# SewoongLab/PLeaS-Merging

Measured on AMD Instinct MI355X. Metric: wall-clock (s): ResNet-101 pair, 100-batch act-match + 400-step PLeaS, 1/8 GPU, lower is better.
Workload: dtype f32

## Files before the change

### include/pleas_hip.h

```cpp
#ifndef PLEAS_HIP_H
#define PLEAS_HIP_H

#include <stddef.h>
#include <stdint.h>

#ifdef __cplusplus
extern "C" {
#endif

#define PLEAS_OK 0
#define PLEAS_EINVAL (-22)
#define PLEAS_ENOMEM (-12)
#define PLEAS_EHIP (-5)

const char* pleas_version(void);
const char* pleas_last_error(void);

#define PLEAS_EPI_INNER 0
#define PLEAS_EPI_NEG_CDIST 1
size_t pleas_gram_ws_bytes(int B, int C, int64_t HW);
int pleas_gram_accum(const float* x, const float* y, int B, int C, int64_t HW, int epilogue, int accumulate,
                     float* acc, void* ws, size_t ws_bytes, void* stream);

typedef struct pleas_gram_node {
// ... 90 lines not shown
    const float* ip;
    const float* w;
    const float* bias;
    const float* o1;
    const float* o2;
    const int32_t* row1;
    const int32_t* row2;
    float* resid;
    int N, Cout, Cin, Hin, Win, KH, KW, stride, pad, Csrc, n_merged;
    float dscale, loss_scale;
    int flags;
} pleas_fwd_layer;
#define PLEAS_FWD_KPOS_MAJOR 1
size_t pleas_fwd_batch_ws_bytes(const pleas_fwd_layer* layers, int n_layers);
int pleas_fwd_plan_lanes(double* form_ms, int* form_lane, int* form_items);
int pleas_fwd_plan_units(const pleas_fwd_layer* layers, int n_layers, const double* form_ms, int* units, int max_units);
int pleas_fwd_batch(const pleas_fwd_layer* layers, int n_layers, float* loss, void* ws, size_t ws_bytes, int ws_fresh,
                    void* stream);
int pleas_conv2d_fwd(const float* x, const float* w, const float* bias, float* y, int N, int Cin, int Hin, int Win, int Cout,
                     int KH, int KW, int stride, int pad, int flags, void* stream);
int pleas_conv2d_bn_act_fwd(const float* x, const float* w, const float* bias, float* y, const float* scale,
                            const float* shift, const float* res, float* z, int relu, int N, int Cin, int Hin, int Win,
                            int Cout, int KH, int KW, int stride, int pad, int flags, void* stream);
int pleas_conv2d_act_fwd(const float* x, const float* w, const float* bias, const float* scale, const float* shift,
                         const float* res, float* z, int relu, int N, int Cin, int Hin, int Win, int Cout, int KH, int KW,
                         int stride, int pad, int flags, void* stream);
size_t pleas_conv2d_bn_stats_ws_bytes(int N, int Cout, int Hout, int Wout, int batches);
int pleas_conv2d_bn_stats_fwd(const float* x, const float* w, const float* bias, float* y, int N, int Cin, int Hin, int Win,
                              int Cout, int KH, int KW, int stride, int pad, int flags, int batches, const float* gamma,
                              const float* beta, double eps, double momentum, float* running_mean, float* running_var,
                              int64_t* num_batches_tracked, float* scale, float* shift, void* ws, size_t ws_bytes, void* stream);
typedef struct pleas_wgrad_layer {
    const float* resid;
    const float* ip;
    float* grad;
    int N, Cout, Cin, Hin, Win, KH, KW, stride, pad;
    int flags;
} pleas_wgrad_layer;
#define PLEAS_WGRAD_ACCUMULATE 1
#define PLEAS_WGRAD_KPOS_MAJOR 2
int pleas_target_residual(const float* out, const float* o1, const float* o2, const int32_t* row1, const int32_t* row2,
                          int n_merged, int N, int C, int Csrc, int64_t HW, float dscale, float* resid, float* partials,
                          int* n_partials, void* stream);
int pleas_target_residual_max_partials(void);
int pleas_loss_final(const float* partials, const int* n_partials, const float* scale, int stride, int n_layers,
                     float* loss, void* stream);
// ... 38 lines not shown
```

### pleas_merging_amd/_lib.py

```python
from __future__ import annotations

import ctypes
import os
from ctypes import POINTER, c_char_p, c_float, c_int, c_int64, c_size_t, c_void_p
from typing import Optional

_LIB: Optional[ctypes.CDLL] = None
LIB_PATH = os.path.join(os.path.dirname(os.path.abspath(__file__)), "csrc", "libpleas_hip.so")

EPI_INNER, EPI_NEG_CDIST = 0, 1
ARITH_FP32, ARITH_SPLIT_BF16, ARITH_SPLIT_BF16_EXACT = 0, 1, 2
LSAP_MAX_N = 4096

SIGNATURES = {
    "pleas_version": (c_char_p, []),
    "pleas_last_error": (c_char_p, []),
    "pleas_gram_ws_bytes": (c_size_t, [c_int, c_int, c_int64]),
    "pleas_gram_accum": (c_int, [c_void_p, c_void_p, c_int, c_int, c_int64, c_int, c_int, c_void_p, c_void_p, c_size_t,
                                 c_void_p]),
    "pleas_lsap_batched": (c_int, [POINTER(c_void_p), POINTER(c_int), c_int, c_int, POINTER(c_void_p), c_void_p]),
    "pleas_lsap_host": (c_int, [c_void_p, c_int, c_int, c_int, c_void_p]),
    "pleas_bottleneck_ws_bytes": (c_size_t, [POINTER(c_int), c_int]),
    "pleas_bottleneck_batched": (c_int, [POINTER(c_void_p), POINTER(c_int), c_int, c_int, POINTER(c_void_p), c_void_p, c_void_p,
                                         c_size_t, c_void_p]),
# ... 30 lines not shown
    "pleas_prof_reset": (None, []),
    "pleas_prof_collect": (c_int, [c_int, POINTER(c_int64), POINTER(ctypes.c_double), POINTER(ctypes.c_double),
                                   POINTER(ctypes.c_double)]),
    "pleas_arith": (None, [c_int]),
    "pleas_arith_get": (c_int, []),
    "pleas_gram_batch_tune": (None, [c_int, c_int]),
    "pleas_target_residual": (c_int, [c_void_p, c_void_p, c_void_p, c_void_p, c_void_p, c_int, c_int, c_int, c_int,
                                      c_int64, c_float, c_void_p, c_void_p, POINTER(c_int), c_void_p]),
    "pleas_target_residual_max_partials": (c_int, []),
    "pleas_loss_final": (c_int, [c_void_p, c_void_p, c_void_p, c_int, c_int, c_void_p, c_void_p]),
    "pleas_cholesky_solve_batched": (c_int, [POINTER(c_void_p), POINTER(c_void_p), POINTER(c_int), POINTER(c_int), c_int,
                                             c_float, c_void_p, c_void_p]),
    "pleas_normal_eq_ws_bytes": (c_size_t, [c_void_p, c_int]),
    "pleas_normal_eq_accum": (c_int, [c_void_p, c_int, c_void_p, c_size_t, c_int, c_void_p]),
    "pleas_normal_eq_finalize": (c_int, [c_void_p, c_int, c_void_p]),
    "pleas_normal_eq_plan_info": (c_int, [c_void_p, c_int, c_void_p]),
    "pleas_fwd_batch_ws_bytes": (c_size_t, [c_void_p, c_int]),
    "pleas_fwd_plan_lanes": (c_int, [c_void_p, c_void_p, c_void_p]),
    "pleas_fwd_plan_units": (c_int, [c_void_p, c_int, c_void_p, c_void_p, c_int]),
    "pleas_allreduce_sum": (c_int, [c_void_p, c_int64, c_void_p, c_void_p]),
    "pleas_fwd_batch": (c_int, [c_void_p, c_int, c_void_p, c_void_p, c_size_t, c_int, c_void_p]),
    "pleas_conv2d_fwd": (c_int, [c_void_p, c_void_p, c_void_p, c_void_p] + [c_int] * 10 + [c_void_p]),
    "pleas_conv2d_bn_act_fwd": (c_int, [c_void_p] * 8 + [c_int] * 11 + [c_void_p]),
    "pleas_conv2d_act_fwd": (c_int, [c_void_p] * 7 + [c_int] * 11 + [c_void_p]),
    "pleas_conv2d_bn_stats_ws_bytes": (c_size_t, [c_int] * 5),
    "pleas_conv2d_bn_stats_fwd": (c_int, [c_void_p] * 4 + [c_int] * 11 + [c_void_p, c_void_p, ctypes.c_double, ctypes.c_double]
                                  + [c_void_p] * 6 + [c_size_t, c_void_p]),
    "pleas_pool_gather": (c_int, [c_void_p, c_void_p, c_void_p, c_int64, c_int, c_int64, c_int, c_void_p]),
    "pleas_top1_count": (c_int, [c_void_p, c_void_p, c_int64, c_int, c_void_p, c_void_p, c_void_p]),
    "pleas_softmax_xent": (c_int, [c_void_p, c_void_p, c_int64, c_int, c_float, c_void_p, c_void_p, c_void_p, c_void_p, c_void_p]),
    "pleas_wgrad_batch_ws_bytes": (c_size_t, [c_void_p, c_int]),
    "pleas_wgrad_batch": (c_int, [c_void_p, c_int, c_void_p, c_size_t, c_int, c_void_p]),
    "pleas_wgrad_plan_info": (c_int, [c_void_p, c_int, POINTER(c_int)]),
    "pleas_gram_batch_ws_bytes": (c_size_t, [c_void_p, c_int, POINTER(c_int), c_int]),
    "pleas_gram_batch": (c_int, [c_void_p, c_int, POINTER(c_void_p), POINTER(c_int), c_int, c_int, c_int, c_void_p,
                                 c_size_t, c_int, c_void_p]),
}


class MergeItem(ctypes.Structure):
    _fields_ = [("w1", c_void_p), ("w2", c_void_p), ("out", c_void_p), ("row1", c_void_p), ("row2", c_void_p),
                ("outer", c_int64), ("inner", c_int64), ("rows_out", c_int), ("rows_src", c_int), ("n_merged", c_int),
                ("sub_stride", c_int), ("sub_h", c_int), ("sub_w", c_int)]


class FwdLayer(ctypes.Structure):
# ... 50 lines not shown
```

### pleas_merging_amd/csrc/conv_fwd.hip

```cpp
#include <algorithm>
#include <mutex>
#include <vector>

#include "fwd_schedule.hpp"
#include "nt_tile.hpp"

namespace pleas {

typedef short s16x4_t __attribute__((ext_vector_type(4)));
typedef short s16x8_t __attribute__((ext_vector_type(8)));

constexpr int fTN = 128;

enum class FwdMode : int { Fit = 0, Conv = 1, ConvImage = 2, Image = 3, ConvStats = 4 };
constexpr int fModes = 5;
constexpr bool fwd_has_target(FwdMode m) { return m == FwdMode::Fit; }
constexpr bool fwd_has_image(FwdMode m) { return m == FwdMode::ConvImage || m == FwdMode::Image; }
constexpr bool fwd_stores_y(FwdMode m) { return m != FwdMode::Image; }
constexpr bool fwd_has_stats(FwdMode m) { return m == FwdMode::ConvStats; }

struct FwdLayerDev {
    const float* ip;
    const float* w;
    const float* bias;
    const float* o1;
    const float* o2;
    const int32_t* row1;
    const int32_t* row2;
    float* resid;
    int Cout, Cin, Hin, Win, Hout, Wout, KH, KW, stride, pad, Csrc, n_merged;
    uint32_t HWo, Ptot, Kd;
    float dscale;
    int variant;
    int part_base;
    int bn_relu;
    const float* bn_scale;
    const float* bn_shift;
    const float* bn_res;
    float* bn_z;
    double* st_part;
    uint32_t st_pb;
};
struct FwdItemDev {
    int layer, tm, tp, slot;
};

template <int TM, bool IMAGE>
struct FwdRowOps {
    int row1[TM / 8], row2[TM / 8];
    float bias[TM / 8];
};
template <int TM>
struct FwdRowOps<TM, true> {
    float scale[TM / 8], shift[TM / 8];
    float bias[TM / 8];
};
template <int TM, FwdMode MODE = FwdMode::Fit>
__device__ __forceinline__ void fwd_load_maps(const FwdLayerDev& L, const int i0, FwdRowOps<TM, fwd_has_image(MODE)>& ops) {
    const int tid = threadIdx.x;
#pragma unroll
    for (int j = 0; j < TM / 8; ++j) {
        const int co = min(i0 + (tid >> 5) + 8 * j, L.Cout - 1);
        if constexpr (fwd_has_image(MODE)) {
            ops.scale[j] = PLEAS_GLOBAL(L.bn_scale)[co];
            ops.shift[j] = PLEAS_GLOBAL(L.bn_shift)[co];
        } else {
            ops.row1[j] = L.row1 ? PLEAS_GLOBAL_I(L.row1)[co] : -1;
            ops.row2[j] = L.row2 ? PLEAS_GLOBAL_I(L.row2)[co] : -1;
        }
        ops.bias[j] = L.bias ? PLEAS_GLOBAL(L.bias)[co] : 0.f;
    }
}

template <int TM, FwdMode MODE = FwdMode::Fit>
__device__ __forceinline__ void fwd_epilogue(const FwdLayerDev& L, const FwdItemDev& it, f32x16 (&acc)[TM / 64][2],
                                             const FwdRowOps<TM, fwd_has_image(MODE)>& ops, float* smem, float* __restrict__ partials) {
    constexpr int MTM = TM / 64;
    constexpr int ROWS = TM / 8, GB = 8, NB = ROWS / GB;
    const int tid = threadIdx.x, lane = tid & 63, wave = tid >> 6;
    const int wm = wave >> 1, wn = wave & 1;
    const int i0 = it.tm * TM;
    const uint32_t p0 = (uint32_t)it.tp * fTN;
    constexpr int EL = 132;
    float* Ct = smem;
    auto spill_acc = [&]() {
#pragma unroll
        for (int sm = 0; sm < MTM; ++sm)
#pragma unroll
            for (int sn = 0; sn < 2; ++sn)
#pragma unroll
                for (int r = 0; r < 16; ++r) {
                    const int lco = wm * (TM / 2) + sm * 32 + (r & 3) + 8 * (r >> 2) + 4 * (lane >> 5);
                    Ct[lco * EL + wn * 64 + sn * 32 + (lane & 31)] = acc[sm][sn][r];
                }
        __syncthreads();
    };
    float sq = 0.f;
    constexpr int SPR = kThreads / TM;
    float st_bias = 0.f;
    if constexpr (fwd_has_stats(MODE)) st_bias = L.bias ? PLEAS_GLOBAL(L.bias)[min(i0 + tid / SPR, L.Cout - 1)] : 0.f;
    const bool vec_ok = (L.HWo % 4 == 0);
    const int pg = (tid & 31) * 4;
    const uint32_t Pg = p0 + pg;
    const bool gin = Pg < L.Ptot;
    const uint32_t gn = gin ? Pg / L.HWo : 0u, gp = gin ? Pg - gn * L.HWo : 0u;
    if (vec_ok) {
        f32x4 ta[NB][GB], tb[NB][GB];
        const uint32_t hw4 = 4u * L.HWo;
        const uint32_t gbase = 4u * (gn * (uint32_t)L.Csrc * L.HWo + gp);
        const uint32_t rbase = 4u * ((gn * (uint32_t)L.Cout + (uint32_t)i0 + (uint32_t)(tid >> 5)) * L.HWo + gp);
        const bool has_res = fwd_has_image(MODE) && L.bn_res != nullptr;
        const char* o1b = reinterpret_cast<const char*>(fwd_has_image(MODE) ? (has_res ? L.bn_res : L.ip) : L.o1);
        const char* o2b = reinterpret_cast<const char*>(L.o2);
        char* rb_ = reinterpret_cast<char*>(L.resid);
        char* zb_ = reinterpret_cast<char*>(L.bn_z);
        auto gather = [&](const int bt) {
#pragma unroll
            for (int u = 0; u < GB; ++u) {
                const int j = bt * GB + u;
                if constexpr (fwd_has_image(MODE)) {
                    const bool live = has_res && gin && i0 + (tid >> 5) + 8 * j < L.Cout;
                    const uint32_t oz = live ? rbase + (uint32_t)(8 * j) * hw4 : 0u;
                    const f32x4 idn = *(const __attribute__((address_space(1))) f32x4*)(o1b + oz);
                    ta[bt][u] = has_res ? idn : f32x4{0.f, 0.f, 0.f, 0.f};
                } else if constexpr (!fwd_has_target(MODE)) {
                    ta[bt][u] = tb[bt][u] = f32x4{0.f, 0.f, 0.f, 0.f};
                } else {
                    const uint32_t oa = (gin && ops.row1[j] >= 0) ? gbase + (uint32_t)ops.row1[j] * hw4 : 0u;
                    const uint32_t ob = (gin && ops.row2[j] >= 0) ? gbase + (uint32_t)ops.row2[j] * hw4 : 0u;
                    ta[bt][u] = *(const __attribute__((address_space(1))) f32x4*)(o1b + oa);
                    tb[bt][u] = *(const __attribute__((address_space(1))) f32x4*)(o2b + ob);
                }
            }
        };
        auto consume = [&](const int bt) {
#pragma unroll
            for (int u = 0; u < GB; ++u) {
                const int j = bt * GB + u;
                const int lco = (tid >> 5) + 8 * j, co = i0 + lco;
                const bool live = gin && co < L.Cout;
                if constexpr (fwd_has_image(MODE)) {
                    const f32x4 o = *reinterpret_cast<const f32x4*>(Ct + lco * EL + pg);
                    f32x4 y, z;
#pragma unroll
                    for (int e = 0; e < 4; ++e) {
                        y[e] = o[e] + ops.bias[j];
                        const float sm = fmaf(y[e], ops.scale[j], ops.shift[j]) + ta[bt][u][e];
                        z[e] = L.bn_relu ? fmaxf(sm, 0.f) : sm;
                    }
                    if (live) {
                        if constexpr (fwd_stores_y(MODE)) *(__attribute__((address_space(1))) f32x4*)(rb_ + (rbase + (uint32_t)(8 * j) * hw4)) = y;
                        *(__attribute__((address_space(1))) f32x4*)(zb_ + (rbase + (uint32_t)(8 * j) * hw4)) = z;
                    }
                } else {
                    const float coef = co < L.n_merged ? 0.5f : 1.0f;
                    const float ca = ops.row1[j] >= 0 ? coef : 0.f, cb = ops.row2[j] >= 0 ? coef : 0.f;
                    const f32x4 o = *reinterpret_cast<const f32x4*>(Ct + lco * EL + pg);
                    f32x4 d;
                    float s4 = 0.f;
#pragma unroll
                    for (int e = 0; e < 4; ++e) {
                        const float dd = (o[e] + ops.bias[j]) - fmaf(tb[bt][u][e], cb, ta[bt][u][e] * ca);
                        s4 = fmaf(dd, dd, s4);
                        d[e] = L.dscale * dd;
                    }
                    sq += live ? s4 : 0.f;
                    if (live) *(__attribute__((address_space(1))) f32x4*)(rb_ + (rbase + (uint32_t)(8 * j) * hw4)) = d;
                }
            }
        };
        gather(0);
        spill_acc();
        if constexpr (NB > 1) gather(1);
        consume(0);
        if constexpr (NB > 1) consume(1);
    } else {
        spill_acc();
#pragma unroll
        for (int j = 0; j < ROWS; ++j) {
            const int lco = (tid >> 5) + 8 * j, co = i0 + lco;
            if (co >= L.Cout || !gin) continue;
            const float coef = co < L.n_merged ? 0.5f : 1.0f;
            const f32x4 o = *reinterpret_cast<const f32x4*>(Ct + lco * EL + pg);
#pragma unroll
            for (int e = 0; e < 4; ++e) {
                const uint32_t Pe = Pg + e;
                if (Pe >= L.Ptot) break;
                const uint32_t n = Pe / L.HWo, p = Pe - n * L.HWo;
                if constexpr (fwd_has_image(MODE)) {
                    const size_t at = ((size_t)n * L.Cout + co) * L.HWo + p;
                    const float y = o[e] + ops.bias[j];
                    const float sm = fmaf(y, ops.scale[j], ops.shift[j]) + (L.bn_res ? PLEAS_GLOBAL(L.bn_res)[at] : 0.f);
                    if constexpr (fwd_stores_y(MODE)) PLEAS_GLOBAL_W(L.resid)[at] = y;
                    PLEAS_GLOBAL_W(L.bn_z)[at] = L.bn_relu ? fmaxf(sm, 0.f) : sm;
                } else {
                    float a = 0.f, b = 0.f;
                    if (ops.row1[j] >= 0) a = PLEAS_GLOBAL(L.o1)[((size_t)n * L.Csrc + ops.row1[j]) * L.HWo + p];
                    if (ops.row2[j] >= 0) b = PLEAS_GLOBAL(L.o2)[((size_t)n * L.Csrc + ops.row2[j]) * L.HWo + p];
                    const float dd = (o[e] + ops.bias[j]) - (a + b) * coef;
                    sq = fmaf(dd, dd, sq);
                    PLEAS_GLOBAL_W(L.resid)[((size_t)n * L.Cout + co) * L.HWo + p] = L.dscale * dd;
                }
            }
        }
    }
    if constexpr (fwd_has_stats(MODE)) {
        constexpr int NCH = 32 / SPR;
        const int r = tid / SPR, q = tid % SPR;
        const int skew = (NCH / 2) * (SPR == 2 ? q : q >> 1);
        const uint32_t bnext = (p0 / L.st_pb + 1u) * L.st_pb;
        const uint32_t n1 = min(L.Ptot - p0, (uint32_t)fTN), n0 = min(bnext - p0, n1);
        double a0 = 0.0, b0 = 0.0, a1 = 0.0, b1 = 0.0;
        const float* row = Ct + r * EL + q * NCH * 4;
        if (n0 == (uint32_t)fTN) {
#pragma unroll
            for (int i = 0; i < NCH; ++i) {
                const f32x4 o = *reinterpret_cast<const f32x4*>(row + 4 * ((i + skew) % NCH));
// ... 518 lines not shown
            } else {
                __syncthreads();
                store_b(0, rb0);
            }
        }
        __syncthreads();
        r1 = r2;
        cb1 = cb2;
    };
    int r = 0;
    int c = 0;
    for (; c + 2 < nchunks; c += 2) {
        const int ra_ = r1;
        step(c, r, ra1, ra0, rb1, rb0);
        const int rb_ = r1;
        step(c + 1, ra_, ra0, ra1, rb0, rb1);
        r = rb_;
    }
    if (c + 1 < nchunks) {
        const int ra_ = r1;
        step(c, r, ra1, ra0, rb1, rb0);
        r = ra_;
    }
    fwd_load_maps<TM, MODE>(L, i0, ops);
    compute((nchunks - 1) & 1, bsel, r);
    __syncthreads();
    fwd_epilogue<TM, MODE>(L, it, acc, ops, smem, partials);
}

struct FwdForm {
    bool flat;
    int tm;
    int sub;
    bool split;
    int occupancy[3];
    double weight;
};
constexpr int fForms = 10;
constexpr FwdForm kFwdForms[fForms] = {
    {false, 128, 4, false, {2, 2, 2}, 2.5}, {false, 64, 4, false, {2, 2, 2}, 2.5},
    {false, 128, 1, false, {2, 2, 2}, 2.5}, {false, 64, 1, false, {2, 2, 2}, 2.5},
    {true, 128, 0, true, {2, 2, 2}, 1.0},   {true, 128, 1, false, {2, 2, 2}, 2.0}, {true, 128, 2, true, {2, 2, 2}, 1.0},
    {true, 64, 0, true, {2, 3, 3}, 1.0},    {true, 64, 1, false, {2, 2, 2}, 2.0},  {true, 64, 2, true, {2, 3, 3}, 1.0},
};
constexpr int fwd_form_of(int variant) {
    if (variant & 8) return ((variant & 1) ? 7 : 4) + ((variant >> 4) & 3);
    return variant & 3;
}
constexpr bool fwd_forms_match_variants() {
    for (int f = 0; f < fForms; ++f) {
// ... 18 lines not shown
}
template <int FORM, int SPLIT, FwdMode MODE>
__global__ __launch_bounds__(kThreads, kFwdForms[FORM].occupancy[SPLIT]) void conv2d_fwd_kernel(const FwdLayerDev L, const int tms) {
    extern __shared__ __attribute__((aligned(16))) float smem[];
    const FwdItemDev it{0, (int)(blockIdx.x % (unsigned)tms), (int)(blockIdx.x / (unsigned)tms), 0};
    constexpr FwdForm F = kFwdForms[FORM];
    static_assert(!fwd_has_target(MODE), "the fit has its own kernel: tables of layers and items, loss partials");
    if constexpr (F.flat) fwd_flat_tile<F.tm, F.sub, SPLIT, MODE>(L, it, smem, nullptr);
    else fwd_tile<F.tm, F.sub, MODE>(L, it, smem, nullptr);
}
struct FwdFormKernels {
    void (*batch[3])(const FwdLayerDev*, const FwdItemDev*, float*);
    void (*conv2d[fModes][3])(const FwdLayerDev, const int);
};
template <int FORM>
static constexpr FwdFormKernels fwd_form_kernels() {
    constexpr int S = kFwdForms[FORM].split ? 1 : 0, S9 = kFwdForms[FORM].split ? 2 : 0;
    using M = FwdMode;
    return {{fwd_batch_kernel<FORM, 0>, fwd_batch_kernel<FORM, S>, fwd_batch_kernel<FORM, S9>},
            {{nullptr, nullptr, nullptr},
             {conv2d_fwd_kernel<FORM, 0, M::Conv>, conv2d_fwd_kernel<FORM, S, M::Conv>, conv2d_fwd_kernel<FORM, S9, M::Conv>},
             {conv2d_fwd_kernel<FORM, 0, M::ConvImage>, conv2d_fwd_kernel<FORM, S, M::ConvImage>, conv2d_fwd_kernel<FORM, S9, M::ConvImage>},
             {conv2d_fwd_kernel<FORM, 0, M::Image>, conv2d_fwd_kernel<FORM, S, M::Image>, conv2d_fwd_kernel<FORM, S9, M::Image>},
             {conv2d_fwd_kernel<FORM, 0, M::ConvStats>, conv2d_fwd_kernel<FORM, S, M::ConvStats>, conv2d_fwd_kernel<FORM, S9, M::ConvStats>}}};
}
static const FwdFormKernels kFwdKernels[fForms] = {fwd_form_kernels<0>(), fwd_form_kernels<1>(), fwd_form_kernels<2>(), fwd_form_kernels<3>(),
                                                   fwd_form_kernels<4>(), fwd_form_kernels<5>(), fwd_form_kernels<6>(), fwd_form_kernels<7>(),
                                                   fwd_form_kernels<8>(), fwd_form_kernels<9>()};
constexpr int fLanes = 3;
static SideStreams<fLanes> g_fwd_side;

struct FwdLossDev {
    int begin, count;
    float scale;
    int pad;
};
__global__ __launch_bounds__(64) void fwd_loss_kernel(const float* __restrict__ partials, const FwdLossDev* __restrict__ ld,
                                                      float* __restrict__ loss) {
    const FwdLossDev d = ld[blockIdx.x];
    double s = 0.0;
    for (int i = threadIdx.x; i < d.count; i += 64) s += (double)partials[d.begin + i];
#pragma unroll
    for (int off = 32; off >= 1; off >>= 1) s += __shfl_xor(s, off);
    if (threadIdx.x == 0) loss[blockIdx.x] = (float)(s * (double)d.scale);
}

constexpr int fPtrBatch = 56;
// ... 203 lines not shown
        units[4 * i + 1] = tmp.units[i].begin;
        units[4 * i + 2] = tmp.units[i].count;
        units[4 * i + 3] = tmp.units[i].lane;
    }
    return (int)tmp.units.size();
}

extern "C" size_t pleas_fwd_batch_ws_bytes(const pleas_fwd_layer* layers, int n_layers) {
    if (!layers || n_layers <= 0) return 0;
    FwdPlan tmp;
    if (build_fwd_plan(tmp, layers, n_layers) != PLEAS_OK) return 0;
    return tmp.total;
}

struct Conv2dCall {
    FwdMode mode;
    const float *x, *w, *bias;
    float* y;
    int N, Cin, Hin, Win, Cout, KH, KW, stride, pad, flags;
    void* stream;
    const float *scale = nullptr, *shift = nullptr, *res = nullptr;
    float* z = nullptr;
    int relu = 0;
};
struct Conv2dPlan { FwdLayerDev d; size_t lds = 0; int TM = 128; };

static int conv2d_describe(const Conv2dCall& c, Conv2dPlan& p) {
    FwdLayerDev& d = p.d;
    if (!c.x || !c.w || (!c.y && fwd_stores_y(c.mode))) return bad_arg("conv2d_fwd: null pointer");
    if (((uintptr_t)c.w & 15) != 0 || ((uintptr_t)c.x & 15) != 0)
        return bad_arg(fwd_has_stats(c.mode) ? "conv2d_bn_stats_fwd: x and w must be 16-byte aligned" : "conv2d_fwd: x and w must be 16-byte aligned");
    if (fwd_has_image(c.mode) && ((((uintptr_t)c.y | (uintptr_t)c.z | (uintptr_t)c.res) & 15) != 0))
        return bad_arg("conv2d_bn_act_fwd: y, z and res must be 16-byte aligned");
    pleas_fwd_layer l{};
    l.N = c.N; l.Cout = c.Cout; l.Cin = c.Cin; l.Hin = c.Hin; l.Win = c.Win; l.KH = c.KH; l.KW = c.KW; l.stride = c.stride; l.pad = c.pad;
    l.Csrc = 1; l.dscale = 1.f; l.flags = c.flags;
    d = FwdLayerDev{};
    if (const int rc = fwd_describe(l, d, p.lds, p.TM); rc != PLEAS_OK) return rc;
    d.ip = c.x; d.w = c.w; d.bias = c.bias; d.o1 = c.x; d.o2 = c.x; d.resid = c.y;
    d.bn_scale = c.scale; d.bn_shift = c.shift; d.bn_res = c.res; d.bn_z = c.z; d.bn_relu = c.relu ? 1 : 0;
    return PLEAS_OK;
}

static int conv2d_enqueue(const Conv2dCall& c, const Conv2dPlan& p) {
    const FwdLayerDev& d = p.d;
    const int tms = (int)ceil_div(c.Cout, p.TM), tps = (int)ceil_div((int64_t)d.Ptot, fTN);
    const dim3 grid((unsigned)((int64_t)tms * tps));
    hipStream_t st = (hipStream_t)c.stream;
    const double out_floats = (double)c.Cout * d.Ptot;
    ProfScope prof(kProfConv2d, 2.0 * c.Cout * (double)d.Kd * (double)d.Ptot,
                   ((double)c.Cin * c.N * c.Hin * c.Win + out_floats * ((c.mode == FwdMode::ConvImage ? 2.0 : 1.0) + (c.res ? 1.0 : 0.0))) * sizeof(float), st);
    hipLaunchKernelGGL(kFwdKernels[fwd_form_of(d.variant)].conv2d[(int)c.mode][arith_mode()], grid, dim3(kThreads), p.lds, st, d, tms);
    PLEAS_LAUNCH_CHECK("conv2d_fwd_kernel");
    return PLEAS_OK;
}

static int conv2d_launch(const Conv2dCall& c) {
    Conv2dPlan p;
    if (const int rc = conv2d_describe(c, p); rc != PLEAS_OK) return rc;
    return conv2d_enqueue(c, p);
}

extern "C" int pleas_conv2d_fwd(const float* x, const float* w, const float* bias, float* y, int N, int Cin, int Hin, int Win,
                                int Cout, int KH, int KW, int stride, int pad, int flags, void* stream_) {
    return conv2d_launch(Conv2dCall{FwdMode::Conv, x, w, bias, y, N, Cin, Hin, Win, Cout, KH, KW, stride, pad, flags, stream_});
}

extern "C" int pleas_conv2d_bn_act_fwd(const float* x, const float* w, const float* bias, float* y, const float* scale,
                                       const float* shift, const float* res, float* z, int relu, int N, int Cin, int Hin,
                                       int Win, int Cout, int KH, int KW, int stride, int pad, int flags, void* stream_) {
    if (!scale || !shift || !z) return bad_arg("conv2d_bn_act_fwd: null pointer");
    return conv2d_launch(Conv2dCall{FwdMode::ConvImage, x, w, bias, y, N, Cin, Hin, Win, Cout, KH, KW, stride, pad, flags, stream_,
                                    scale, shift, res, z, relu});
}

extern "C" int pleas_conv2d_act_fwd(const float* x, const float* w, const float* bias, const float* scale, const float* shift,
                                    const float* res, float* z, int relu, int N, int Cin, int Hin, int Win, int Cout, int KH,
                                    int KW, int stride, int pad, int flags, void* stream_) {
    if (!scale || !shift || !z) return bad_arg("conv2d_act_fwd: null pointer");
    return conv2d_launch(Conv2dCall{FwdMode::Image, x, w, bias, nullptr, N, Cin, Hin, Win, Cout, KH, KW, stride, pad, flags, stream_,
                                    scale, shift, res, z, relu});
}

static size_t conv_bn_stats_head(int Cout, int batches) { return (size_t)batches * Cout * 4; }

extern "C" size_t pleas_conv2d_bn_stats_ws_bytes(int N, int Cout, int Hout, int Wout, int batches) {
    if (N <= 0 || Cout <= 0 || Hout <= 0 || Wout <= 0 || batches <= 0) return 0;
    const int64_t tiles = ceil_div((int64_t)N * Hout * Wout, fTN);
    return (conv_bn_stats_head(Cout, batches) + (size_t)tiles * 2 * Cout * 2) * sizeof(double);
}

extern "C" int pleas_conv2d_bn_stats_fwd(const float* x, const float* w, const float* bias, float* y, int N, int Cin, int Hin, int Win,
                                         int Cout, int KH, int KW, int stride, int pad, int flags, int batches, const float* gamma,
                                         const float* beta, double eps, double momentum, float* running_mean, float* running_var,
                                         int64_t* num_batches_tracked, float* scale, float* shift, void* ws, size_t ws_bytes,
                                         void* stream_) {
// ... 135 lines not shown
```

### pleas_merging_amd/hip_ops.py

```python
from __future__ import annotations

import contextlib
import ctypes
import math
import os
import threading
from typing import List, Optional, Sequence, Tuple

import numpy as np
import torch

from . import _lib
from ._lib import ARITH_FP32, ARITH_SPLIT_BF16, ARITH_SPLIT_BF16_EXACT, EPI_INNER, EPI_NEG_CDIST, PleasHipError, check


class _Pinned(threading.local):

    depth = 0
    handle = 0


_PINNED = _Pinned()


# ... 745 lines not shown


def column_sum(x: torch.Tensor, out: torch.Tensor) -> torch.Tensor:
    _need_gpu(x, out)
    if x.dim() != 2 or not x.is_contiguous() or x.shape[0] < 1 or x.shape[1] < 1:
        raise PleasHipError("column_sum: x must be a contiguous, non-empty [N, C] tensor, got %s" % (tuple(x.shape),))
    if out.device != x.device or out.numel() != x.shape[1] or not out.is_contiguous():
        raise PleasHipError("column_sum: out must hold %d contiguous floats on x's device" % x.shape[1])
    check(_lib.lib().pleas_column_sum(x.data_ptr(), x.shape[0], x.shape[1], out.data_ptr(), _stream()), "pleas_column_sum")
    return out


def conv2d_bn_act(x: torch.Tensor, w: torch.Tensor, bias: Optional[torch.Tensor], stride: int, pad: int, kpos_major: bool,
                  scale: torch.Tensor, shift: torch.Tensor, res: Optional[torch.Tensor], relu: bool):
    operands, geometry, out_shape = _conv_call("conv2d_bn_act", x, w, bias, stride, pad, kpos_major, scale, shift)
    image = _image_operands("conv2d_bn_act", x, scale, shift, res, out_shape)
    y = torch.empty(out_shape, dtype=torch.float32, device=x.device)
    z = torch.empty_like(y)
    check(_lib.lib().pleas_conv2d_bn_act_fwd(*operands, y.data_ptr(), *image, z.data_ptr(), 1 if relu else 0, *geometry, _stream()),
          "pleas_conv2d_bn_act_fwd")
    return y, z


CONV_MAX_OUTPUT, CONV_MAX_PIXELS = 1 << 30, 1 << 31


def conv2d_sample_split(N: int, per_sample_out: int, pixels: int, limit: int = CONV_MAX_OUTPUT, align: int = 1) -> List[Tuple[int, int]]:
    if N <= 0:
        return []
    most = min((limit - 1) // per_sample_out, (CONV_MAX_PIXELS - 1) // pixels) // align * align
    if most <= 0:
        raise PleasHipError("conv2d_act: one sample (%d output elements, %d pixels) exceeds the per-call limit" % (per_sample_out, pixels))
    groups = -(-N // align)
    calls = -(-groups // (most // align))
    base, extra = divmod(groups, calls)
    parts, at = [], 0
    for i in range(calls):
        n = min((base + (1 if i < extra else 0)) * align, N - at)
        parts.append((at, n))
        at += n
    return parts


def conv2d_act(x: torch.Tensor, w: torch.Tensor, bias: Optional[torch.Tensor], stride: int, pad: int, kpos_major: bool,
               scale: torch.Tensor, shift: torch.Tensor, res: Optional[torch.Tensor], relu: bool,
               _limit: int = CONV_MAX_OUTPUT) -> torch.Tensor:
# ... 278 lines not shown
```

### pleas_merging_amd/methods/activation_matching.py

```python
from __future__ import annotations

import os

from typing import Callable, Dict, Iterable, List, Optional, Tuple

import torch
import torch.fx
from torch import nn

from ..core.solvers import hip_solve_lsa, hip_solve_minimax_assignment
from ..core.utils import Axis, Permutation, PermutationSpec
from .. import hip_ops
from ..hip_ops import cross_features_cdist, cross_features_inner_product

_FUSED_EPILOGUE = {}


def _register_fused():
    from .. import hip_ops

    _FUSED_EPILOGUE[hip_ops.cross_features_cdist] = hip_ops.EPI_NEG_CDIST
    _FUSED_EPILOGUE[hip_ops.cross_features_inner_product] = hip_ops.EPI_INNER


# ... 125 lines not shown
    return gm


def _bn_chains(traced: _Trace, model1: nn.Module, model2: nn.Module):
    from .source_forward import _foldable, _foldable_train, bn_chain

    mods1, mods2 = dict(model1.named_modules()), dict(model2.named_modules())
    at, absorbed, claimed = {}, set(), set()
    for node in traced.graph.nodes:
        if (node.op != "call_module" or len(node.args) != 1 or node.kwargs
                or not all(_foldable(m) or _foldable_train(m) for m in (mods1.get(node.target), mods2.get(node.target)))):
            continue
        add, relu, res = bn_chain(node, mods1, bare_add=True, claimed=claimed)
        last = relu or add or node
        at[last] = (node, add, relu, res)
        absorbed |= {n for n in (node, add, relu) if n is not None and n is not last}
    return at, absorbed


def _build_split_twin(model1: nn.Module, model2: nn.Module, axes: Iterable[Axis], emit: Callable, streams: _SideStream,
                      fuse_bn: bool = False, emit_derived: Optional[Callable] = None):
    import operator

    from .source_forward import _foldable, _train_fold, fold_bn

    traced = _Trace(model1)
    submods = dict(traced.named_modules())
    root = nn.ModuleList([model1, model2])
    chains, absorbed = _bn_chains(traced, model1, model2) if fuse_bn else ({}, set())
    want_early: Dict[str, List[int]] = {}
    for ax in axes:
        want_early.setdefault(ax.key, []).append(ax.axis)
    derivable = set()
    if emit_derived is not None:
        for bn, _add, _relu, _res in chains.values():
            src = bn.args[0]
            if isinstance(src, torch.fx.Node) and src.op not in ("placeholder", "output") and src not in absorbed \
                    and want_early.get(bn.name) == [1] and 1 in want_early.get(src.name, ()):
                derivable.add(bn)
    fold_attrs: Tuple[dict, dict] = ({}, {})
    want: Dict[str, List[int]] = {}
    for ax in axes:
        if ax.axis not in want.setdefault(ax.key, []):
            want[ax.key].append(ax.axis)
    twin = torch.fx.Graph()
    env = ({}, {})
    shared = {}
    for node in traced.graph.nodes:
        if node.op == "placeholder":
            shared[node] = twin.placeholder(node.target)
    ret = None
    for side in (1, 0):
        first = True
        for node in traced.graph.nodes:
            if node.op == "placeholder":
                env[side][node] = shared[node]
                if side == 1 and first:
                    env[side][node] = _node(twin, "call_function", streams.fork, (shared[node],), "fork")
                    first = False
                continue
            if node.op == "output":
                (ret,) = node.args
                continue
            if node in chains:
                bn, add, relu, res = chains[node]
                mod = (model1, model2)[side].get_submodule(bn.target)
                if _foldable(mod):
                    names = ["_pleas_%s_%d_%s" % (kind, side, bn.name) for kind in ("scale", "shift")]
                    for nm_, buf in zip(names, fold_bn(mod)):
                        root.register_buffer(nm_, buf, persistent=False)
                    attrs = (_node(twin, "get_attr", names[0], (), "bn_scale"), _node(twin, "get_attr", names[1], (), "bn_shift"))
                else:
                    fold = _node(twin, "call_function", _train_fold(mod, "%d_%s" % (side, bn.name), streams), (env[side][bn.args[0]],), "bn_stats")
                    attrs = (_node(twin, "call_function", operator.getitem, (fold, 0), "bn_scale"),
                             _node(twin, "call_function", operator.getitem, (fold, 1), "bn_shift"))
                fold_attrs[side][bn] = attrs
                fused = _node(twin, "call_function", hip_ops.bn_act_tracked,
                              (env[side][bn.args[0]], attrs[0], attrs[1], env[side][res] if res is not None else None,
                               relu is not None, bn not in derivable), "bn_chain")
                for slot, member in enumerate((bn, add, relu)):
                    if member is not None:
                        env[side][member] = _node(twin, "call_function", operator.getitem, (fused, slot), "chain_out")
                continue
            if node in absorbed:
                continue
            new = _out_of_place(twin, node, lambda n, side=side: env[side][n], submods)
            if new is not None:
                env[side][node] = new
                continue
            own = _own_conv(twin, node, side, (model1, model2)[side], env[side])
            if own is not None:
                env[side][node] = own
                continue
            new = twin.node_copy(node, lambda n, side=side: env[side][n])
            if node.op in ("call_module", "get_attr"):
                new.target = "%d.%s" % (side, node.target)
            env[side][node] = new
        if side == 1:
            _node(twin, "call_function", streams.back, (), "back")
    _node(twin, "call_function", streams.join, (), "join")
    cross: Dict[Tuple[str, int], torch.fx.Node] = {}
    for node in traced.graph.nodes:
        for a in want.get(node.name, ()) if node.op not in ("placeholder", "output") else ():
            if node in derivable:
                cross[node.name, a] = emit_derived(twin, node.name, node.args[0].name, a, fold_attrs[0][node], fold_attrs[1][node])
            else:
                cross[node.name, a] = emit(twin, node.name, a, env[0][node], env[1][node])
# ... 262 lines not shown
```

### pleas_merging_amd/methods/source_forward.py

```python
from __future__ import annotations

import operator
import os
from typing import Callable, Optional

import torch
import torch.fx
import torch.nn.functional as F
from torch import nn

from .. import hip_ops


SOURCE_CONV = os.environ.get("PLEAS_SOURCE_CONV", "all")
SOURCE_CONV_BN = os.environ.get("PLEAS_SOURCE_CONV_BN", "1")


def own_conv_ok(mod: nn.Module, mode: Optional[str] = None) -> bool:
    mode = SOURCE_CONV if mode is None else mode
    if mode == "vendor" or type(mod) is not nn.Conv2d:
        return False
    if not (mod.groups == 1 and mod.dilation == (1, 1) and mod.padding_mode == "zeros" and isinstance(mod.padding, tuple)
            and mod.stride[0] == mod.stride[1] and mod.padding[0] == mod.padding[1] and mod.kernel_size[0] == mod.kernel_size[1]):
        return False
    k = mod.kernel_size[0]
    return mod.weight.dtype == torch.float32 and k * k <= 64 and (k > 1 or mode == "all")


def _own_input(x, w, dims: int = 4):
    if (not x.is_cuda or x.dtype != torch.float32 or x.dim() != dims or not w.is_cuda
            or (torch.is_grad_enabled() and (x.requires_grad or w.requires_grad))):
        return None
    return x if x.is_contiguous() else x.contiguous()


def _fire_hooks(mod: nn.Module, x, y):
    replaced = False
    for hook in list(mod._forward_hooks.values()):
# ... 52 lines not shown
    def __call__(self, x, scale, shift, res, relu):
        own, conv = self.own, self.own.conv
        xc = self._fused_input(x, scale, res)
        if xc is None:
            return _bn_act(own(x), scale, shift, res, relu)
        y, z = hip_ops.conv2d_bn_act(xc, own.weight(), conv.bias, own.stride, own.pad, own.kpos, scale, shift, res, relu)
        if own.fire_hooks and conv._forward_hooks:
            y, replaced = _fire_hooks(conv, x, y)
            if replaced:
                return _bn_act(y, scale, shift, res, relu)
        return z


class HipConvAct(HipConvBnAct):

    suffix = "_act"

    def __call__(self, x, scale, shift, res, relu):
        own, conv = self.own, self.own.conv
        xc = None if own.fire_hooks and conv._forward_hooks else self._fused_input(x, scale, res)
        if xc is None:
            return super().__call__(x, scale, shift, res, relu)
        return hip_ops.conv2d_act(xc, own.weight(), conv.bias, own.stride, own.pad, own.kpos, scale, shift, res, relu)


class PoolGather:

    def __init__(self):
        self.src = None
        self.__name__ = self.__qualname__ = "pool_gather"

    def __call__(self, x):
        if not x.is_cuda or x.dtype != torch.float32 or x.dim() != 4:
            y = torch.flatten(F.adaptive_avg_pool2d(x, 1), 1)
            return y if self.src is None else y[:, self.src.long()]
        return hip_ops.pool_gather(x, self.src)


class HipLinear:

    def __init__(self, fc: nn.Linear, tag: str):
        self.fc = fc
        self.__name__ = self.__qualname__ = "hip_linear_%s" % tag

    def __call__(self, x):
        fc, w = self.fc, self.fc.weight
# ... 363 lines not shown
```

Before: 5.832.

## Fuse conv with tracked BN/residual/ReLU chain in twin activation-matching graph

Adds a conv kernel mode that writes the pre-BN output, the residual sum and the ReLU output in one epilogue. The twin-graph builder now routes eligible conv→BN→add→ReLU chains through this fused op instead of a separate conv plus bn_act_tracked pass. This removes a full read and rewrite of each activation between the two passes. For one tile configuration it also delays loading the BN maps until after the accumulators are spilled, to ease register pressure. In exchange the kernel table gains a sixth mode, which adds compile size and register risk.

Measured after the change: 5.789 (median of 6 runs). About the same (-0.7%).

```diff
diff --git a/include/pleas_hip.h b/include/pleas_hip.h
--- a/include/pleas_hip.h
+++ b/include/pleas_hip.h
@@ -136,6 +136,9 @@
 int pleas_conv2d_bn_act_fwd(const float* x, const float* w, const float* bias, float* y, const float* scale,
                             const float* shift, const float* res, float* z, int relu, int N, int Cin, int Hin, int Win,
                             int Cout, int KH, int KW, int stride, int pad, int flags, void* stream);
+int pleas_conv2d_bn_act_sum_fwd(const float* x, const float* w, const float* bias, float* y, const float* scale,
+                                const float* shift, const float* res, float* sum, float* z, int N, int Cin, int Hin, int Win,
+                                int Cout, int KH, int KW, int stride, int pad, int flags, void* stream);
 int pleas_conv2d_act_fwd(const float* x, const float* w, const float* bias, const float* scale, const float* shift,
                          const float* res, float* z, int relu, int N, int Cin, int Hin, int Win, int Cout, int KH, int KW,
                          int stride, int pad, int flags, void* stream);
diff --git a/pleas_merging_amd/_lib.py b/pleas_merging_amd/_lib.py
--- a/pleas_merging_amd/_lib.py
+++ b/pleas_merging_amd/_lib.py
@@ -76,6 +76,7 @@
     "pleas_fwd_batch": (c_int, [c_void_p, c_int, c_void_p, c_void_p, c_size_t, c_int, c_void_p]),
     "pleas_conv2d_fwd": (c_int, [c_void_p, c_void_p, c_void_p, c_void_p] + [c_int] * 10 + [c_void_p]),
     "pleas_conv2d_bn_act_fwd": (c_int, [c_void_p] * 8 + [c_int] * 11 + [c_void_p]),
+    "pleas_conv2d_bn_act_sum_fwd": (c_int, [c_void_p] * 9 + [c_int] * 10 + [c_void_p]),
     "pleas_conv2d_act_fwd": (c_int, [c_void_p] * 7 + [c_int] * 11 + [c_void_p]),
     "pleas_conv2d_bn_stats_ws_bytes": (c_size_t, [c_int] * 5),
     "pleas_conv2d_bn_stats_fwd": (c_int, [c_void_p] * 4 + [c_int] * 11 + [c_void_p, c_void_p, ctypes.c_double, ctypes.c_double]
diff --git a/pleas_merging_amd/csrc/conv_fwd.hip b/pleas_merging_amd/csrc/conv_fwd.hip
--- a/pleas_merging_amd/csrc/conv_fwd.hip
+++ b/pleas_merging_amd/csrc/conv_fwd.hip
@@ -12,10 +12,11 @@
 
 constexpr int fTN = 128;
 
-enum class FwdMode : int { Fit = 0, Conv = 1, ConvImage = 2, Image = 3, ConvStats = 4 };
-constexpr int fModes = 5;
+enum class FwdMode : int { Fit = 0, Conv = 1, ConvImage = 2, Image = 3, ConvStats = 4, ConvImageSum = 5 };
+constexpr int fModes = 6;
 constexpr bool fwd_has_target(FwdMode m) { return m == FwdMode::Fit; }
-constexpr bool fwd_has_image(FwdMode m) { return m == FwdMode::ConvImage || m == FwdMode::Image; }
+constexpr bool fwd_has_image(FwdMode m) { return m == FwdMode::ConvImage || m == FwdMode::Image || m == FwdMode::ConvImageSum; }
+constexpr bool fwd_has_sum(FwdMode m) { return m == FwdMode::ConvImageSum; }
 constexpr bool fwd_stores_y(FwdMode m) { return m != FwdMode::Image; }
 constexpr bool fwd_has_stats(FwdMode m) { return m == FwdMode::ConvStats; }
 
@@ -38,7 +39,10 @@
     const float* bn_shift;
     const float* bn_res;
     float* bn_z;
-    double* st_part;
+    union {
+        double* st_part;
+        float* bn_sum;
+    };
     uint32_t st_pb;
 };
 struct FwdItemDev {
@@ -72,15 +76,18 @@
     }
 }
 
-template <int TM, FwdMode MODE = FwdMode::Fit>
+template <int TM, FwdMode MODE = FwdMode::Fit, bool LATE_OPS = false>
 __device__ __forceinline__ void fwd_epilogue(const FwdLayerDev& L, const FwdItemDev& it, f32x16 (&acc)[TM / 64][2],
                                              const FwdRowOps<TM, fwd_has_image(MODE)>& ops, float* smem, float* __restrict__ partials) {
+    static_assert(!LATE_OPS || fwd_has_image(MODE), "the fit's gathers need the block maps before the accumulators are spilled");
     constexpr int MTM = TM / 64;
     constexpr int ROWS = TM / 8, GB = 8, NB = ROWS / GB;
     const int tid = threadIdx.x, lane = tid & 63, wave = tid >> 6;
     const int wm = wave >> 1, wn = wave & 1;
     const int i0 = it.tm * TM;
     const uint32_t p0 = (uint32_t)it.tp * fTN;
+    FwdRowOps<TM, fwd_has_image(MODE)> late;
+    const FwdRowOps<TM, fwd_has_image(MODE)>& rops = LATE_OPS ? late : ops;
     constexpr int EL = 132;
     float* Ct = smem;
     auto spill_acc = [&]() {
@@ -109,11 +116,13 @@
         const uint32_t hw4 = 4u * L.HWo;
         const uint32_t gbase = 4u * (gn * (uint32_t)L.Csrc * L.HWo + gp);
         const uint32_t rbase = 4u * ((gn * (uint32_t)L.Cout + (uint32_t)i0 + (uint32_t)(tid >> 5)) * L.HWo + gp);
-        const bool has_res = fwd_has_image(MODE) && L.bn_res != nullptr;
+        const bool has_res = fwd_has_sum(MODE) || (fwd_has_image(MODE) && L.bn_res != nullptr);
         const char* o1b = reinterpret_cast<const char*>(fwd_has_image(MODE) ? (has_res ? L.bn_res : L.ip) : L.o1);
         const char* o2b = reinterpret_cast<const char*>(L.o2);
         char* rb_ = reinterpret_cast<char*>(L.resid);
         char* zb_ = reinterpret_cast<char*>(L.bn_z);
+        char* sb_ = nullptr;
+        if constexpr (fwd_has_sum(MODE)) sb_ = reinterpret_cast<char*>(L.bn_sum);
         auto gather = [&](const int bt) {
 #pragma unroll
             for (int u = 0; u < GB; ++u) {
@@ -141,15 +150,21 @@
                 const bool live = gin && co < L.Cout;
                 if constexpr (fwd_has_image(MODE)) {
                     const f32x4 o = *reinterpret_cast<const f32x4*>(Ct + lco * EL + pg);
-                    f32x4 y, z;
+                    f32x4 y, z, s;
 #pragma unroll
                     for (int e = 0; e < 4; ++e) {
-                        y[e] = o[e] + ops.bias[j];
-                        const float sm = fmaf(y[e], ops.scale[j], ops.shift[j]) + ta[bt][u][e];
-                        z[e] = L.bn_relu ? fmaxf(sm, 0.f) : sm;
+                        y[e] = o[e] + rops.bias[j];
+                        const float sm = fmaf(y[e], rops.scale[j], rops.shift[j]) + ta[bt][u][e];
+                        if constexpr (fwd_has_sum(MODE)) {
+                            s[e] = sm;
+                            z[e] = fmaxf(sm, 0.f);
+                        } else {
+                            z[e] = L.bn_relu ? fmaxf(sm, 0.f) : sm;
+                        }
                     }
                     if (live) {
                         if constexpr (fwd_stores_y(MODE)) *(__attribute__((address_space(1))) f32x4*)(rb_ + (rbase + (uint32_t)(8 * j) * hw4)) = y;
+                        if constexpr (fwd_has_sum(MODE)) *(__attribute__((address_space(1))) f32x4*)(sb_ + (rbase + (uint32_t)(8 * j) * hw4)) = s;
                         *(__attribute__((address_space(1))) f32x4*)(zb_ + (rbase + (uint32_t)(8 * j) * hw4)) = z;
                     }
                 } else {
@@ -171,11 +186,13 @@
         };
         gather(0);
         spill_acc();
+        if constexpr (LATE_OPS) fwd_load_maps<TM, MODE>(L, i0, late);
         if constexpr (NB > 1) gather(1);
         consume(0);
         if constexpr (NB > 1) consume(1);
     } else {
         spill_acc();
+        if constexpr (LATE_OPS) fwd_load_maps<TM, MODE>(L, i0, late);
 #pragma unroll
         for (int j = 0; j < ROWS; ++j) {
             const int lco = (tid >> 5) + 8 * j, co = i0 + lco;
@@ -189,10 +206,15 @@
                 const uint32_t n = Pe / L.HWo, p = Pe - n * L.HWo;
                 if constexpr (fwd_has_image(MODE)) {
                     const size_t at = ((size_t)n * L.Cout + co) * L.HWo + p;
-                    const float y = o[e] + ops.bias[j];
-                    const float sm = fmaf(y, ops.scale[j], ops.shift[j]) + (L.bn_res ? PLEAS_GLOBAL(L.bn_res)[at] : 0.f);
+                    const float y = o[e] + rops.bias[j];
+                    const float sm = fmaf(y, rops.scale[j], rops.shift[j]) + (L.bn_res ? PLEAS_GLOBAL(L.bn_res)[at] : 0.f);
                     if constexpr (fwd_stores_y(MODE)) PLEAS_GLOBAL_W(L.resid)[at] = y;
-                    PLEAS_GLOBAL_W(L.bn_z)[at] = L.bn_relu ? fmaxf(sm, 0.f) : sm;
+                    if constexpr (fwd_has_sum(MODE)) {
+                        PLEAS_GLOBAL_W(L.bn_sum)[at] = sm;
+                        PLEAS_GLOBAL_W(L.bn_z)[at] = fmaxf(sm, 0.f);
+                    } else {
+                        PLEAS_GLOBAL_W(L.bn_z)[at] = L.bn_relu ? fmaxf(sm, 0.f) : sm;
+                    }
                 } else {
                     float a = 0.f, b = 0.f;
                     if (ops.row1[j] >= 0) a = PLEAS_GLOBAL(L.o1)[((size_t)n * L.Csrc + ops.row1[j]) * L.HWo + p];
@@ -757,10 +779,11 @@
         step(c, r, ra1, ra0, rb1, rb0);
         r = ra_;
     }
-    fwd_load_maps<TM, MODE>(L, i0, ops);
+    constexpr bool LATE = fwd_has_sum(MODE) && SPLIT == 1 && TM == 128 && KIND == 0;
+    if constexpr (!LATE) fwd_load_maps<TM, MODE>(L, i0, ops);
     compute((nchunks - 1) & 1, bsel, r);
     __syncthreads();
-    fwd_epilogue<TM, MODE>(L, it, acc, ops, smem, partials);
+    fwd_epilogue<TM, MODE, LATE>(L, it, acc, ops, smem, partials);
 }
 
 struct FwdForm {
@@ -825,7 +848,8 @@
              {conv2d_fwd_kernel<FORM, 0, M::Conv>, conv2d_fwd_kernel<FORM, S, M::Conv>, conv2d_fwd_kernel<FORM, S9, M::Conv>},
              {conv2d_fwd_kernel<FORM, 0, M::ConvImage>, conv2d_fwd_kernel<FORM, S, M::ConvImage>, conv2d_fwd_kernel<FORM, S9, M::ConvImage>},
              {conv2d_fwd_kernel<FORM, 0, M::Image>, conv2d_fwd_kernel<FORM, S, M::Image>, conv2d_fwd_kernel<FORM, S9, M::Image>},
-             {conv2d_fwd_kernel<FORM, 0, M::ConvStats>, conv2d_fwd_kernel<FORM, S, M::ConvStats>, conv2d_fwd_kernel<FORM, S9, M::ConvStats>}}};
+             {conv2d_fwd_kernel<FORM, 0, M::ConvStats>, conv2d_fwd_kernel<FORM, S, M::ConvStats>, conv2d_fwd_kernel<FORM, S9, M::ConvStats>},
+             {conv2d_fwd_kernel<FORM, 0, M::ConvImageSum>, conv2d_fwd_kernel<FORM, S, M::ConvImageSum>, conv2d_fwd_kernel<FORM, S9, M::ConvImageSum>}}};
 }
 static const FwdFormKernels kFwdKernels[fForms] = {fwd_form_kernels<0>(), fwd_form_kernels<1>(), fwd_form_kernels<2>(), fwd_form_kernels<3>(),
                                                    fwd_form_kernels<4>(), fwd_form_kernels<5>(), fwd_form_kernels<6>(), fwd_form_kernels<7>(),
@@ -1075,6 +1099,7 @@
     const float *scale = nullptr, *shift = nullptr, *res = nullptr;
     float* z = nullptr;
     int relu = 0;
+    float* sum = nullptr;
 };
 struct Conv2dPlan { FwdLayerDev d; size_t lds = 0; int TM = 128; };
 
@@ -1085,6 +1110,7 @@
         return bad_arg(fwd_has_stats(c.mode) ? "conv2d_bn_stats_fwd: x and w must be 16-byte aligned" : "conv2d_fwd: x and w must be 16-byte aligned");
     if (fwd_has_image(c.mode) && ((((uintptr_t)c.y | (uintptr_t)c.z | (uintptr_t)c.res) & 15) != 0))
         return bad_arg("conv2d_bn_act_fwd: y, z and res must be 16-byte aligned");
+    if (fwd_has_sum(c.mode) && ((uintptr_t)c.sum & 15) != 0) return bad_arg("conv2d_bn_act_sum_fwd: sum must be 16-byte aligned");
     pleas_fwd_layer l{};
     l.N = c.N; l.Cout = c.Cout; l.Cin = c.Cin; l.Hin = c.Hin; l.Win = c.Win; l.KH = c.KH; l.KW = c.KW; l.stride = c.stride; l.pad = c.pad;
     l.Csrc = 1; l.dscale = 1.f; l.flags = c.flags;
@@ -1092,6 +1118,7 @@
     if (const int rc = fwd_describe(l, d, p.lds, p.TM); rc != PLEAS_OK) return rc;
     d.ip = c.x; d.w = c.w; d.bias = c.bias; d.o1 = c.x; d.o2 = c.x; d.resid = c.y;
     d.bn_scale = c.scale; d.bn_shift = c.shift; d.bn_res = c.res; d.bn_z = c.z; d.bn_relu = c.relu ? 1 : 0;
+    if (fwd_has_sum(c.mode)) d.bn_sum = c.sum;
     return PLEAS_OK;
 }
 
@@ -1102,7 +1129,7 @@
     hipStream_t st = (hipStream_t)c.stream;
     const double out_floats = (double)c.Cout * d.Ptot;
     ProfScope prof(kProfConv2d, 2.0 * c.Cout * (double)d.Kd * (double)d.Ptot,
-                   ((double)c.Cin * c.N * c.Hin * c.Win + out_floats * ((c.mode == FwdMode::ConvImage ? 2.0 : 1.0) + (c.res ? 1.0 : 0.0))) * sizeof(float), st);
+                   ((double)c.Cin * c.N * c.Hin * c.Win + out_floats * ((c.mode == FwdMode::ConvImage ? 2.0 : c.mode == FwdMode::ConvImageSum ? 3.0 : 1.0) + (c.res ? 1.0 : 0.0))) * sizeof(float), st);
     hipLaunchKernelGGL(kFwdKernels[fwd_form_of(d.variant)].conv2d[(int)c.mode][arith_mode()], grid, dim3(kThreads), p.lds, st, d, tms);
     PLEAS_LAUNCH_CHECK("conv2d_fwd_kernel");
     return PLEAS_OK;
@@ -1125,6 +1152,14 @@
     if (!scale || !shift || !z) return bad_arg("conv2d_bn_act_fwd: null pointer");
     return conv2d_launch(Conv2dCall{FwdMode::ConvImage, x, w, bias, y, N, Cin, Hin, Win, Cout, KH, KW, stride, pad, flags, stream_,
                                     scale, shift, res, z, relu});
+}
+
+extern "C" int pleas_conv2d_bn_act_sum_fwd(const float* x, const float* w, const float* bias, float* y, const float* scale,
+                                           const float* shift, const float* res, float* sum, float* z, int N, int Cin, int Hin,
+                                           int Win, int Cout, int KH, int KW, int stride, int pad, int flags, void* stream_) {
+    if (!scale || !shift || !res || !sum || !z) return bad_arg("conv2d_bn_act_sum_fwd: null pointer");
+    return conv2d_launch(Conv2dCall{FwdMode::ConvImageSum, x, w, bias, y, N, Cin, Hin, Win, Cout, KH, KW, stride, pad, flags, stream_,
+                                    scale, shift, res, z, 1, sum});
 }
 
 extern "C" int pleas_conv2d_act_fwd(const float* x, const float* w, const float* bias, const float* scale, const float* shift,
diff --git a/pleas_merging_amd/hip_ops.py b/pleas_merging_amd/hip_ops.py
--- a/pleas_merging_amd/hip_ops.py
+++ b/pleas_merging_amd/hip_ops.py
@@ -791,6 +791,19 @@
     return y, z
 
 
+def conv2d_bn_act_sum(x: torch.Tensor, w: torch.Tensor, bias: Optional[torch.Tensor], stride: int, pad: int, kpos_major: bool,
+                      scale: torch.Tensor, shift: torch.Tensor, res: torch.Tensor):
+    operands, geometry, out_shape = _conv_call("conv2d_bn_act_sum", x, w, bias, stride, pad, kpos_major, scale, shift)
+    if res is None:
+        raise PleasHipError("conv2d_bn_act_sum: the identity is required (conv2d_bn_act takes a chain without one)")
+    image = _image_operands("conv2d_bn_act_sum", x, scale, shift, res, out_shape)
+    y = torch.empty(out_shape, dtype=torch.float32, device=x.device)
+    s, z = torch.empty_like(y), torch.empty_like(y)
+    check(_lib.lib().pleas_conv2d_bn_act_sum_fwd(*operands, y.data_ptr(), *image, s.data_ptr(), z.data_ptr(), *geometry, _stream()),
+          "pleas_conv2d_bn_act_sum_fwd")
+    return y, s, z
+
+
 CONV_MAX_OUTPUT, CONV_MAX_PIXELS = 1 << 30, 1 << 31
 
 
diff --git a/pleas_merging_amd/methods/activation_matching.py b/pleas_merging_amd/methods/activation_matching.py
--- a/pleas_merging_amd/methods/activation_matching.py
+++ b/pleas_merging_amd/methods/activation_matching.py
@@ -171,7 +171,8 @@
                       fuse_bn: bool = False, emit_derived: Optional[Callable] = None):
     import operator
 
-    from .source_forward import _foldable, _train_fold, fold_bn
+    from . import source_forward
+    from .source_forward import HipConv, HipConvBnTracked, _foldable, _train_fold, fold_bn, own_conv_ok
 
     traced = _Trace(model1)
     submods = dict(traced.named_modules())
@@ -187,6 +188,21 @@
             if isinstance(src, torch.fx.Node) and src.op not in ("placeholder", "output") and src not in absorbed \
                     and want_early.get(bn.name) == [1] and 1 in want_early.get(src.name, ()):
                 derivable.add(bn)
+    riding: Tuple[dict, dict] = ({}, {})
+    if source_forward.TWIN_CONV_BN == "1":
+        for last, (bn, _add, _relu, _res) in chains.items():
+            src = bn.args[0]
+            if not (isinstance(src, torch.fx.Node) and src.op == "call_module" and len(src.args) == 1 and not src.kwargs
+                    and len(src.users) == 1 and src not in absorbed and src not in chains and (bn in derivable or last is bn)):
+                continue
+            for side, model in enumerate((model1, model2)):
+                try:
+                    conv = model.get_submodule(src.target)
+                except AttributeError:
+                    continue
+                if own_conv_ok(conv) and _foldable(model.get_submodule(bn.target)):
+                    riding[side][last] = (src, conv)
+    ridden = tuple({src for src, _conv in riding[side].values()} for side in (0, 1))
     fold_attrs: Tuple[dict, dict] = ({}, {})
     want: Dict[str, List[int]] = {}
     for ax in axes:
@@ -224,6 +240,15 @@
                     attrs = (_node(twin, "call_function", operator.getitem, (fold, 0), "bn_scale"),
                              _node(twin, "call_function", operator.getitem, (fold, 1), "bn_shift"))
                 fold_attrs[side][bn] = attrs
+                if node in riding[side]:
+                    src, conv = riding[side][node]
+                    fused = _node(twin, "call_function", HipConvBnTracked(HipConv(conv, "%d_%s" % (side, src.name))),
+                                  (env[side][src.args[0]], attrs[0], attrs[1], env[side][res] if res is not None else None,
+                                   relu is not None), "hip_conv_bn_chain")
+                    for slot, member in enumerate((src, bn, add, relu)):
+                        if member is not None:
+                            env[side][member] = _node(twin, "call_function", operator.getitem, (fused, slot), "chain_out")
+                    continue
                 fused = _node(twin, "call_function", hip_ops.bn_act_tracked,
                               (env[side][bn.args[0]], attrs[0], attrs[1], env[side][res] if res is not None else None,
                                relu is not None, bn not in derivable), "bn_chain")
@@ -232,6 +257,8 @@
                         env[side][member] = _node(twin, "call_function", operator.getitem, (fused, slot), "chain_out")
                 continue
             if node in absorbed:
+                continue
+            if node in ridden[side]:
                 continue
             new = _out_of_place(twin, node, lambda n, side=side: env[side][n], submods)
             if new is not None:
diff --git a/pleas_merging_amd/methods/source_forward.py b/pleas_merging_amd/methods/source_forward.py
--- a/pleas_merging_amd/methods/source_forward.py
+++ b/pleas_merging_amd/methods/source_forward.py
@@ -14,6 +14,7 @@
 
 SOURCE_CONV = os.environ.get("PLEAS_SOURCE_CONV", "all")
 SOURCE_CONV_BN = os.environ.get("PLEAS_SOURCE_CONV_BN", "1")
+TWIN_CONV_BN = os.environ.get("PLEAS_TWIN_CONV_BN", "1")
 
 
 def own_conv_ok(mod: nn.Module, mode: Optional[str] = None) -> bool:
@@ -112,6 +113,29 @@
         if xc is None:
             return super().__call__(x, scale, shift, res, relu)
         return hip_ops.conv2d_act(xc, own.weight(), conv.bias, own.stride, own.pad, own.kpos, scale, shift, res, relu)
+
+
+class HipConvBnTracked(HipConvBnAct):
+
+    suffix = "_bn_tracked"
+
+    def __call__(self, x, scale, shift, res, relu):
+        own, conv = self.own, self.own.conv
+        xc = self._fused_input(x, scale, res)
+        if xc is None:
+            y = own(x)
+            return (y,) + tuple(hip_ops.bn_act_tracked(y, scale, shift, res, relu, False))
+        if res is not None and relu:
+            y, sm, act = hip_ops.conv2d_bn_act_sum(xc, own.weight(), conv.bias, own.stride, own.pad, own.kpos, scale, shift, res)
+            out = (None, sm, act)
+        else:
+            y, z = hip_ops.conv2d_bn_act(xc, own.weight(), conv.bias, own.stride, own.pad, own.kpos, scale, shift, res, relu)
+            out = (None, z, None) if res is not None else ((None, None, z) if relu else (z, None, None))
+        if own.fire_hooks and conv._forward_hooks:
+            y, replaced = _fire_hooks(conv, x, y)
+            if replaced:
+                return (y,) + tuple(hip_ops.bn_act_tracked(y, scale, shift, res, relu, False))
+        return (y,) + out
 
 
 class PoolGather:
```
